# qzs634/Probabilistic-Multiplanar-Unet

Measured on AMD Instinct MI355X. Metric: 2D slices/sec fwd+bwd, 256×256×1 batch32 U-Net; Dice vs ref, higher is better.
Workload: dtype fp32; 1 GPU; c2: UNet(n_channels=1, n_classes=1, num_filters=[64, 128, 256, 512, 1024]), 256x256x1 slices, fwd+BCE+bwd+clip(0.1)+SGD(0.9) per step, fp32; global_batch=32, per_gpu_batch=32, parallelism=dp1

## Files before the change

include/pmunet_hip.h:

```cpp
#ifndef PMUNET_HIP_H
#define PMUNET_HIP_H
#include <stddef.h>
#ifdef __cplusplus
extern "C" {
#endif

#define PMU_ABI_VERSION 1

enum { PMU_OK = 0, PMU_ERR_ARG = 1001 };

enum {
  PMU_SRC_RAW = 0,
  PMU_SRC_BNRELU = 1,
  PMU_SRC_BNBWD = 2
};
enum { PMU_POOL_NONE = 0, PMU_POOL_MAX2 = 1, PMU_POOL_AVG2CEIL = 2 };
enum { PMU_DT_X_BF16 = 1, PMU_DT_Z_BF16 = 2 };

typedef struct pmu_src {
  const float* x;
  const float* z;
  const float* coef;
  int mode, pool;
  int C, H, W;
  int off_h, off_w;
  int dtype;
} pmu_src;

typedef struct pmu_frame {
  pmu_src src[2];
  int nsrc;
  int N, H, W;
} pmu_frame;

size_t pmu_conv3x3_wgrad_ws(int N, int H, int W, int Cin, int Cout);
int pmu_conv3x3_wgrad(const pmu_frame* dz, const pmu_frame* act, int Cout, float* dw,
                      float* ws, size_t ws_bytes, void* stream);

size_t pmu_conv3x3_packed_size_wino(int Cout, int Cin, int dgrad);
int pmu_conv3x3_pack_wino(const float* w, int Cout, int Cin, int dgrad, float* wp, void* stream);
int pmu_conv3x3_tiles_wino(int N, int H, int W);
int pmu_conv3x3_fwd_wino(const pmu_frame* in, const float* wp, const float* bias, int Cout, float* z,
                         float* part, float* tee, void* stream);
int pmu_conv3x3_dgrad_wino(const pmu_frame* dz, const float* wp, int Cin, int Csplit, float* dx0, float* dx1,
                           float* tee, void* stream);
size_t pmu_conv3x3_packed_size_wino2h(int Cout, int Cin, int dgrad);
int pmu_conv3x3_pack_wino2h(const float* w, int Cout, int Cin, int dgrad, float* wp, void* stream);
int pmu_conv3x3_tiles_wino2h(int N, int H, int W);
int pmu_conv3x3_fwd_wino2h(const float* xt, int Cin, int N, int H, int W, const float* wp, const float* bias,
                           int Cout, float* z, float* part, void* stream);
int pmu_conv3x3_dgrad_wino2h(const float* dzt, int Cout, int N, int H, int W, const float* wp, int Cin,
                             int Csplit, float* dx0, float* dx1, void* stream);
int pmu_conv3x3_dgrad_wino2h_bnr(const float* dzt, int Cout, int N, int H, int W, const float* wp, int Cin,
                                 float* dx, const float* z, const float* coef, const float* mean,
                                 const float* invstd, float* part, void* stream);
size_t pmu_conv3x3_packed_size_wino4(int Cout, int Cin, int dgrad);
int pmu_conv3x3_pack_wino4(const float* w, int Cout, int Cin, int dgrad, float* wp, void* stream);
int pmu_conv3x3_tiles_wino4(int N, int H, int W);
int pmu_conv3x3_dgrad_wino4(const float* dzt, int Cout, int N, int H, int W, const float* wp, int Cin,
                            int Csplit, float* dx0, float* dx1, void* stream);
int pmu_conv3x3_dgrad_wino4_bnr(const float* dzt, int Cout, int N, int H, int W, const float* wp, int Cin,
                                float* dx, const float* z, const float* coef, const float* mean,
                                const float* invstd, float* part, void* stream);
size_t pmu_conv3x3_wgrad_ws_wino(int N, int H, int W, int Cin, int Cout);
int pmu_conv3x3_wgrad_wino(const float* dzt, const float* xt, int N, int H, int W, int Cout, int Cin,
                           float* dw, float* ws, size_t ws_bytes, void* stream);

size_t pmu_conv3x3_packed_size_bf16(int Cout, int Cin, int dgrad);
int pmu_conv3x3_pack_bf16(const float* w, int Cout, int Cin, int dgrad, unsigned short* wp, void* stream);
int pmu_conv3x3_tiles(int N, int H, int W);
int pmu_conv3x3_fwd_bf16(const pmu_frame* in, const unsigned short* wp, const float* bias, int Cout,
                         float* z, float* part, unsigned short* tee, void* stream);
int pmu_conv3x3_dgrad_bf16(const pmu_frame* dz, const unsigned short* wp, int Cin, int Csplit,
                           float* dx0, float* dx1, unsigned short* tee, void* stream);

size_t pmu_conv3x3_packed_size_raw(int Cout, int Cin, int dgrad);
int pmu_conv3x3_pack_raw(const float* w, int Cout, int Cin, int dgrad, unsigned short* wp, void* stream);
int pmu_conv3x3_fwd_raw(const unsigned short* xt, int Cp, int N, int H, int W, const unsigned short* wp,
                        const float* bias, int Cout, float* z, float* part, void* stream);
int pmu_conv3x3_tiles_raw(int N, int H, int W, int Cout);
int pmu_conv3x3_dgrad_raw(const unsigned short* dzt, int Cp, int N, int H, int W, const unsigned short* wp,
                          int Cin, int Csplit, float* dx0, float* dx1, void* stream);
int pmu_conv3x3_dma_ok(int H, int W, int Cp, int NOUT, int split);
int pmu_conv3x3_tiles_dma(int N, int H, int W, int Cout, int Cp);
size_t pmu_conv3x3_packed_size_dma(int Cout, int Cin, int dgrad);
int pmu_conv3x3_pack_dma(const float* w, int Cout, int Cin, int dgrad, unsigned short* wp, void* stream);
int pmu_conv3x3_fwd_dma(const unsigned short* xt, int Cp, int N, int H, int W, const unsigned short* wp,
                        const float* bias, int Cout, float* z, float* part, void* stream);
int pmu_conv3x3_dgrad_dma(const unsigned short* dzt, int Cp, int N, int H, int W, const unsigned short* wp,
                          int Cin, int Csplit, float* dx0, float* dx1, void* stream);
int pmu_conv3x3_dgrad_dma_x1b(const unsigned short* dzt, int Cp, int N, int H, int W, const unsigned short* wp,
                              int Cin, int Csplit, float* dx0, float* dx1, unsigned short* dx1b, void* stream);
int pmu_conv3x3_dgrad_dma_x1b_sum(const unsigned short* dzt, int Cp, int N, int H, int W, const unsigned short* wp,
                                  int Cin, int Csplit, float* dx0, unsigned short* dx1b, float* part, void* stream);
size_t pmu_convT2x2_dbias_rows_ws(int Cout);
int pmu_convT2x2_dbias_rows(const float* part, int R, long long ld, int Cout, float* dbias, float* ws, void* stream);
int pmu_conv3x3_dgrad_dma_bnr(const unsigned short* dzt, int Cp, int N, int H, int W, const unsigned short* wp,
                              int Cin, float* dx, const float* z, const float* coef, const float* mean,
                              const float* invstd, float* part, void* stream);
int pmu_conv3x3_dgrad_dma_dxb(const unsigned short* dzt, int Cp, int N, int H, int W, const unsigned short* wp,
                              int Cin, int Csplit, unsigned short* dx0, float* dx1, void* stream);
// ... 230 lines not shown
```

probabilistic-multiplanar-unet_amd/csrc/conv3x3_wino2h.hip:

```cpp
#include <string.h>
#include <stdlib.h>
#include "pmu_common.h"
#include "pmu_lds.h"

namespace {

constexpr int TX = 8, TY = 8;
constexpr int OW = 2 * TX, OH = 2 * TY;
constexpr int HW = OW + 2, HH = OH + 2;
constexpr int BK = 8;
constexpr int GP = 20;
constexpr int ROWF = 208;
constexpr int ROWU = ROWF / 4;
constexpr int A_FLOATS = HH * ROWF;
[[maybe_unused]] constexpr int NC = 16;
constexpr int NCP = 16;
constexpr int A_UNITS = A_FLOATS / 4;

__host__ __device__ constexpr int u_swz(int row) { return (row >> 2) & 3; }

template <int CO_>
struct W2Cfg {
  static constexpr int CO = CO_;
  static constexpr int NT = 16 * CO_;
  static constexpr int NW = NT / 64;
  static constexpr int U_FLOATS = BK * CO_ * NCP;
  static constexpr int STAGE = A_FLOATS + U_FLOATS;
  static constexpr int NGL = (A_UNITS + NT - 1) / NT;
  static constexpr int UGL = (U_FLOATS / 4 + NT - 1) / NT;
  static constexpr int RED_FLOATS = NW * 16 * 2;
  static constexpr int XB_FLOATS = NW * 2 * 4 * 64;
  static_assert(U_FLOATS % (4 * 64) == 0, "U of whole wave DMA instructions");
  static_assert(XB_FLOATS <= STAGE, "exchange round fits a stage");
  static_assert((2 * STAGE + RED_FLOATS) * 4 <= 160 * 1024, "LDS");
};

struct W2Args {
  const float* x;
  const float* wp;
  const float* bias;
  float* out0;
  float* out1;
  float* part;
  int H, W, KC, NOUT, split, bw, bh, nco, cpb;
  int N;
  const float* bz;
  const float* bcoef;
  const float* bmean;
  const float* binv;
};

__device__ __forceinline__ void wino2_u(const float (&g)[3][3], float (&u)[16]) {
  float t[4][3];
  for (int b = 0; b < 3; ++b) {
    t[0][b] = g[0][b];
    t[1][b] = 0.5f * (g[0][b] + g[1][b] + g[2][b]);
    t[2][b] = 0.5f * (g[0][b] - g[1][b] + g[2][b]);
    t[3][b] = g[2][b];
  }
  for (int a = 0; a < 4; ++a) {
    u[4 * a + 0] = t[a][0];
    u[4 * a + 1] = 0.5f * (t[a][0] + t[a][1] + t[a][2]);
    u[4 * a + 2] = 0.5f * (t[a][0] - t[a][1] + t[a][2]);
    u[4 * a + 3] = t[a][2];
  }
}

template <int CO>
__device__ __forceinline__ void pack_wino2h_body(const float* __restrict__ w, int Cout, int Cin, int dgrad,
                                                 float* __restrict__ wp, int bid, int nblk) {
  const int NOUT = dgrad ? Cin : Cout, KC = dgrad ? Cout : Cin;
  const int nch = (KC + BK - 1) / BK, ncob = (NOUT + CO - 1) / CO;
  const long long total = (long long)ncob * nch * BK * CO;
  for (long long e = (long long)bid * blockDim.x + threadIdx.x; e < total; e += (long long)nblk * blockDim.x) {
    const int col = (int)(e % CO);
    long long r = e / CO;
    const int kl = (int)(r % BK); r /= BK;
    const int ch = (int)(r % nch);
    const int jb = (int)(r / nch);
    const int j = jb * CO + col, k = ch * BK + kl;
    float g[3][3];
    for (int a = 0; a < 3; ++a)
      for (int b = 0; b < 3; ++b) {
        float v = 0.f;
        if (j < NOUT && k < KC)
          v = dgrad ? w[((long long)k * Cin + j) * 9 + (2 - a) * 3 + (2 - b)] : w[((long long)j * Cin + k) * 9 + a * 3 + b];
        g[a][b] = v;
      }
    float u[16];
    wino2_u(g, u);
    float* dst = wp + (((long long)jb * nch + ch) * BK + kl) * (CO * NCP) + col * NCP;
    const int sw = u_swz(kl * CO + col);
    for (int q = 0; q < 4; ++q)
      *reinterpret_cast<float4*>(dst + 4 * (q ^ sw)) = make_float4(u[4 * q], u[4 * q + 1], u[4 * q + 2], u[4 * q + 3]);
  }
}
template <int CO>
// ... 259 lines not shown
        float* rowp = dst + (long long)((long long)n * a.H + min(hh, a.H - 1)) * a.W * ld;
#pragma unroll
        for (int q = 0; q < 2; ++q) {
          const int ww = ow + q;
          const float v = P[2 * p + q] + xv[2 * p + q] + bias;
          const bool ok = jok && hh < a.H && ww < a.W;
          if (!DGRAD) {
            const float m = ok ? v : 0.f;
            s1 += m;
            s2 = fmaf(m, m, s2);
          } else if (BNR) {
            const float zz = zt[2 * p + q];
            const float g = (ok && fmaf(zz, bsc, bsh) > 0.f) ? v : 0.f;
            s1 += g;
            s2 = fmaf(g, (zz - bmu) * bis, s2);
          }
          if (!ok) continue;
          PMU_DCHECK((((long long)n * a.H + hh) * a.W + ww) < (long long)a.N * a.H * a.W && j < a.NOUT, PMU_DBG_OUTPUT);
          rowp[(unsigned)(ww * ld)] = v;
        }
      }
    }
  }
  if (a.part) {
    s1 += __shfl_xor(s1, 16, 64);
    s2 += __shfl_xor(s2, 16, 64);
    s1 += __shfl_xor(s1, 32, 64);
    s2 += __shfl_xor(s2, 32, 64);
    if (lane < 16) {
      red[(wave * 16 + lane) * 2 + 0] = s1;
      red[(wave * 16 + lane) * 2 + 1] = s2;
    }
    __syncthreads();
    if (tid < CO) {
      const int jj = j0 + tid, cgg = tid >> 5, hf = (tid >> 4) & 1, l = tid & 15;
      if (jj < a.NOUT) {
        float t1 = 0.f, t2 = 0.f;
#pragma unroll
        for (int g = 0; g < 4; ++g) {
          const int wv = g + 4 * hf + 8 * cgg;
          t1 += red[(wv * 16 + l) * 2 + 0];
          t2 += red[(wv * 16 + l) * 2 + 1];
        }
        PMU_DCHECK(spatial < (long long)a.N * a.bh * a.bw, PMU_DBG_WORKSPACE);
        a.part[((long long)spatial * 2 + 0) * a.NOUT + jj] = t1;
        a.part[((long long)spatial * 2 + 1) * a.NOUT + jj] = t2;
      }
    }
  }
  __syncthreads();
}

struct W2Block {
  int n, h0, w0, cob0, spatial, nchunks, npass;
  unsigned gin, gzero;
};

template <bool DGRAD, bool BNR, int CH, int CO_, bool P64>
__device__ __forceinline__ void wino2h_main(const W2Args& a, const W2Block& B, const unsigned (&goff)[W2Cfg<CO_>::NGL],
                                            float* smem) {
  using C = W2Cfg<CO_>;
  constexpr int CO = C::CO, NT = C::NT, NGL = C::NGL, UGL = C::UGL, U_FLOATS = C::U_FLOATS, STAGE = C::STAGE;
  float* red = smem + 2 * STAGE;
  const int tid = threadIdx.x, lane = tid & 63, wave = tid >> 6;
  const int nchunks = B.nchunks, total = B.npass * nchunks;
  const float* wsrc = a.wp + (long long)B.cob0 * nchunks * U_FLOATS;
  const unsigned uoff = 16u * tid;
  const int wave_off = wave * 256;
  const unsigned gin = B.gin;
#define PMU_FETCH2(GI, BUF)                                                                                 \
  {                                                                                                        \
    const int p_ = (GI) / nchunks;                                                                         \
    const int c_ = (GI) - p_ * nchunks;                                                                    \
    const int cs_ = ((B.cob0 + p_) & 1) ? nchunks - 1 - c_ : c_;                                           \
    const int k0_ = cs_ * BK;                                                                              \
    PMU_DCHECK(k0_ + BK <= a.KC, PMU_DBG_OPERAND);                                                         \
    float* b_ = (BUF);                                                                                     \
    const char* xb_ = reinterpret_cast<const char*>(a.x + k0_);                                            \
    _Pragma("unroll") for (int r = 0; r < NGL; ++r)                                                        \
      if ((gin >> r) & 1u) PMU_GLDS(xb_ + goff[r], b_ + 4 * (r * NT) + wave_off)                           \
    const char* s_ = reinterpret_cast<const char*>(wsrc + ((long long)p_ * nchunks + cs_) * U_FLOATS) + uoff; \
    float* d_ = b_ + A_FLOATS + wave_off;                                                                  \
    _Pragma("unroll") for (int r = 0; r < UGL; ++r)                                                        \
      if (r * NT * 4 + (wave + 1) * 256 <= U_FLOATS) PMU_GLDS(s_ + 16 * NT * r, d_ + 4 * NT * r)          \
  }
  const int t = lane & 15, kk = lane >> 4, tg = wave & 3, cg = wave >> 3;
  const int pbase = 2 * (2 * tg + (t >> 3)) * ROWF + GP * (t & 7) + 2 * kk;
  const int ubase = A_FLOATS + (2 * kk * CO + 32 * cg + t) * NCP;
  static_assert(CO % 16 == 0, "u_swz of every row a lane reads is (t >> 2) & 3");
  const unsigned uoff0 = 4u * ubase + 16u * ((2 * CH) ^ ((t >> 2) & 3));
  f32x4 acc[2][8];
#pragma unroll
  for (int h = 0; h < 2; ++h)
#pragma unroll
    for (int c = 0; c < 8; ++c) acc[h][c] = f32x4{0.f, 0.f, 0.f, 0.f};

  PMU_FETCH2(0, smem)
  asm volatile("s_waitcnt vmcnt(0)" ::: "memory");
  __syncthreads();
  for (int p = 0; p < B.npass; ++p) {
    const int j0 = (B.cob0 + p) * CO;
    const int jb = j0 + 32 * cg + 16 * CH + t;
    const float bias = (!DGRAD && a.bias && jb < a.NOUT) ? a.bias[jb] : 0.f;
    int gi = p * nchunks;
    for (int ch = 0; ch < nchunks; ++ch, ++gi) {
      float* cur = smem + (gi & 1) * STAGE;
      if (gi + 1 < total) PMU_FETCH2(gi + 1, smem + ((gi + 1) & 1) * STAGE)
      const unsigned pa = lds_addr(cur + pbase), ua0 = lds_addr(cur) + uoff0, ua1 = ua0 ^ 16u;
      if constexpr (P64) {
        w2_pair<CH, CO>(pa, ua0, acc);
      } else {
        w2_step<CH>(pa, ua0, ua1, acc);
        w2_step<CH>(pa + 4, ua0 + CO * NCP * 4, ua1 + CO * NCP * 4, acc);
      }
      asm volatile("s_waitcnt vmcnt(0)" ::: "memory");
      __syncthreads();
    }
    int ne = B.n, h0e = B.h0, w0e = B.w0;
    asm volatile("" : "+s"(ne), "+s"(h0e), "+s"(w0e));
    float* xb = smem + ((gi - 1) & 1) * STAGE;
    wino2h_epilogue<DGRAD, BNR, CH, CO>(a, ne, h0e, w0e, j0, B.spatial, acc, xb, red, bias);
    if (p + 1 < B.npass) {
#pragma unroll
      for (int r = 0; r < NGL; ++r)
        if ((B.gzero >> r) & 1u) *reinterpret_cast<float4*>(xb + 4 * (r * NT + tid)) = make_float4(0.f, 0.f, 0.f, 0.f);
      __syncthreads();
    }
#pragma unroll
    for (int h = 0; h < 2; ++h)
#pragma unroll
      for (int c = 0; c < 8; ++c) acc[h][c] = f32x4{0.f, 0.f, 0.f, 0.f};
  }
#undef PMU_FETCH2
}

template <bool DGRAD, bool BNR, int CO_, bool P64 = true>
__global__ __launch_bounds__(16 * CO_, CO_ == 32 ? 4 : 1) void conv3x3_wino2h_kernel(W2Args a) {
  using C = W2Cfg<CO_>;
  constexpr int NT = C::NT, NGL = C::NGL, STAGE = C::STAGE;
  __shared__ __attribute__((aligned(64))) float smem[2 * STAGE + C::RED_FLOATS];
  static_assert(A_FLOATS % 16 == 0 && STAGE % 16 == 0, "U rows 64-B aligned (ua1 = ua0 ^ 16)");
  const int tid = threadIdx.x;
  const int lb = pmu_xcd_block(blockIdx.x, gridDim.x);
  const int ncog = (a.nco + a.cpb - 1) / a.cpb;
  W2Block B;
  B.cob0 = (lb % ncog) * a.cpb;
  int sp = lb / ncog;
  B.spatial = sp;
  const int bx = sp % a.bw; sp /= a.bw;
  const int by = sp % a.bh;
  B.n = sp / a.bh;
  B.h0 = by * OH;
  B.w0 = bx * OW;
  const int KC = a.KC;
  B.nchunks = KC / BK;
  B.npass = a.cpb < a.nco - B.cob0 ? a.cpb : a.nco - B.cob0;
  PMU_DCHECK(B.n < a.N && B.cob0 < a.nco, PMU_DBG_GRID);
  unsigned goff[NGL];
  unsigned gin = 0u, gzero = 0u;
#pragma unroll
  for (int r = 0; r < NGL; ++r) {
    const int u = r * NT + tid;
    const int hr = u / ROWU, wu = u - hr * ROWU;
    const int g = wu / 5, w5 = wu - 5 * g;
    const int px = 2 * g + (w5 >> 1);
    const bool data = u < A_UNITS && w5 < 4 && px < HW;
    const int h = B.h0 - 1 + hr, w = B.w0 - 1 + px;
    const bool in = data && h >= 0 && w >= 0 && h < a.H && w < a.W;
    goff[r] = in ? (unsigned)(((((long long)B.n * a.H + h) * a.W + w) * KC + 4 * (w5 & 1)) * 4) : 0u;
    PMU_DCHECK(!in || (((long long)B.n * a.H + h) * a.W + w) < (long long)a.N * a.H * a.W, PMU_DBG_OPERAND);
    gin |= in ? (1u << r) : 0u;
    gzero |= (data && !in) ? (1u << r) : 0u;
    if (data && !in) {
      *reinterpret_cast<float4*>(smem + 4 * u) = make_float4(0.f, 0.f, 0.f, 0.f);
      *reinterpret_cast<float4*>(smem + STAGE + 4 * u) = make_float4(0.f, 0.f, 0.f, 0.f);
    }
  }
  B.gin = gin;
  B.gzero = gzero;
  if ((tid >> 8) & 1) wino2h_main<DGRAD, BNR, 1, CO_, P64>(a, B, goff, smem);
  else wino2h_main<DGRAD, BNR, 0, CO_, P64>(a, B, goff, smem);
}

static int w2h_co() {
  static const int v = pmu_variant_int("PMU_WINO2H_CO", 64) == 32 ? 32 : 64;
  return v;
}

int launch_wino2h(const float* x, int KC, int N, int H, int W, const float* wp, const float* bias, int NOUT,
                  float* out0, float* out1, int split, float* part, bool dgrad, void* stream,
                 const float* bz = nullptr, const float* bcoef = nullptr, const float* bmean = nullptr,
                 const float* binv = nullptr) {
  const pmu_wino_call c{x, KC, N, H, W, wp, bias, NOUT, out0, out1, split, part, bz, bcoef, bmean, binv};
  const int CO = w2h_co();
  return pmu_wino_launch<W2Args>(c, OW, OH, BK, CO, "PMU_WINO2H_CPB", "PMU_WINO2H_MINWG",
                                 [&](const W2Args& a, long long, dim3 grid) {
    hipStream_t st = (hipStream_t)stream;
    const bool bnr = dgrad && bz;
#ifdef PMU_EXPERIMENTS
    static const int b32 = pmu_variant_int("PMU_WINO2H_B32", 0);
    if (CO == 32 && bnr) hipLaunchKernelGGL((conv3x3_wino2h_kernel<true, true, 32, false>), grid, dim3(512), 0, st, a);
    else if (CO == 32 && dgrad) hipLaunchKernelGGL((conv3x3_wino2h_kernel<true, false, 32, false>), grid, dim3(512), 0, st, a);
    else if (CO == 32) hipLaunchKernelGGL((conv3x3_wino2h_kernel<false, false, 32, false>), grid, dim3(512), 0, st, a);
    else if (b32 && bnr) hipLaunchKernelGGL((conv3x3_wino2h_kernel<true, true, 64, false>), grid, dim3(1024), 0, st, a);
    else if (b32 && dgrad) hipLaunchKernelGGL((conv3x3_wino2h_kernel<true, false, 64, false>), grid, dim3(1024), 0, st, a);
    else if (b32) hipLaunchKernelGGL((conv3x3_wino2h_kernel<false, false, 64, false>), grid, dim3(1024), 0, st, a);
    else
#endif
    if (bnr) hipLaunchKernelGGL((conv3x3_wino2h_kernel<true, true, 64>), grid, dim3(1024), 0, st, a);
    else if (dgrad) hipLaunchKernelGGL((conv3x3_wino2h_kernel<true, false, 64>), grid, dim3(1024), 0, st, a);
    else hipLaunchKernelGGL((conv3x3_wino2h_kernel<false, false, 64>), grid, dim3(1024), 0, st, a);
    PMU_CHECK_LAUNCH();
    return (int)PMU_OK;
  });
}

}

extern "C" int pmu_conv3x3_tiles_wino2h(int N, int H, int W) { return N * pmu_cdiv(H, OH) * pmu_cdiv(W, OW); }

extern "C" size_t pmu_conv3x3_packed_size_wino2h(int Cout, int Cin, int dgrad) {
  const int NOUT = dgrad ? Cin : Cout, KC = dgrad ? Cout : Cin;
  const int CO = w2h_co();
  return (size_t)pmu_cdiv(NOUT, CO) * pmu_cdiv(KC, BK) * (BK * CO * NCP) * sizeof(float);
}

extern "C" int pmu_conv3x3_pack_wino2h(const float* w, int Cout, int Cin, int dgrad, float* wp, void* stream) {
  PMU_REQUIRE(w && wp && Cout > 0 && Cin > 0);
  const long long total = (long long)pmu_conv3x3_packed_size_wino2h(Cout, Cin, dgrad) / sizeof(float) / NCP;
  const int blocks = (int)((total + 255) / 256 < 4096 ? (total + 255) / 256 : 4096);
  hipStream_t st = (hipStream_t)stream;
  const unsigned segs = (unsigned)(pmu_cdiv(Cout, w2h_co()) * pmu_cdiv(Cin, BK));
#ifdef PMU_EXPERIMENTS
  if (w2h_co() == 32 && !dgrad)
    hipLaunchKernelGGL(pack_wino2h_fwd_kernel<32>, dim3(segs), dim3(256), 0, st, w, Cout, Cin, wp);
  else if (w2h_co() == 32)
    hipLaunchKernelGGL(pack_wino2h_kernel<32>, dim3(blocks), dim3(256), 0, st, w, Cout, Cin, dgrad, wp);
  else
#endif
  if (!dgrad) hipLaunchKernelGGL(pack_wino2h_fwd_kernel<64>, dim3(segs), dim3(256), 0, st, w, Cout, Cin, wp);
  else hipLaunchKernelGGL(pack_wino2h_kernel<64>, dim3(blocks), dim3(256), 0, st, w, Cout, Cin, dgrad, wp);
  PMU_CHECK_LAUNCH();
  return PMU_OK;
}

extern "C" int pmu_conv3x3_fwd_wino2h(const float* xt, int Cin, int N, int H, int W, const float* wp, const float* bias,
                                      int Cout, float* z, float* part, void* stream) {
  return launch_wino2h(xt, Cin, N, H, W, wp, bias, Cout, z, nullptr, Cout, part, false, stream);
}

extern "C" int pmu_conv3x3_dgrad_wino2h(const float* dzt, int Cout, int N, int H, int W, const float* wp, int Cin,
                                        int Csplit, float* dx0, float* dx1, void* stream) {
  PMU_REQUIRE(Csplit > 0 && Csplit <= Cin && (Csplit == Cin || dx1));
  return launch_wino2h(dzt, Cout, N, H, W, wp, nullptr, Cin, dx0, dx1, Csplit, nullptr, true, stream);
}

extern "C" int pmu_conv3x3_dgrad_wino2h_bnr(const float* dzt, int Cout, int N, int H, int W, const float* wp, int Cin,
                                            float* dx, const float* z, const float* coef, const float* mean,
                                            const float* invstd, float* part, void* stream) {
  PMU_REQUIRE(z && coef && mean && invstd && part);
  return launch_wino2h(dzt, Cout, N, H, W, wp, nullptr, Cin, dx, nullptr, Cin, part, true, stream, z, coef, mean,
                       invstd);
}

static int pack_wino2h_grid(int Cout, int Cin, int dgrad) {
  if (!dgrad) return pmu_cdiv(Cout, w2h_co()) * pmu_cdiv(Cin, BK);
  const long long total = (long long)pmu_conv3x3_packed_size_wino2h(Cout, Cin, dgrad) / sizeof(float) / NCP;
  return (int)((total + 255) / 256 < 4096 ? (total + 255) / 256 : 4096);
}

extern "C" int pmu_conv3x3_pack_wino2h_blocks(int Cout, int Cin, int dgrad) { return pack_wino2h_grid(Cout, Cin, dgrad); }

extern "C" int pmu_conv3x3_pack_wino2h_multi(const pmu_pack_job* jobs, int njobs, int blocks, int dgrad, void* stream) {
// ... 7 lines not shown
```

probabilistic-multiplanar-unet_amd/csrc/conv3x3_wino4.hip:

```cpp
#include <string.h>
#include <stdlib.h>
#include <utility>
#include "pmu_common.h"
#include "pmu_lds.h"

namespace {

constexpr int TX = 8, TY = 8;
constexpr int OW = 4 * TX, OH = 4 * TY;
constexpr int HW = OW + 2, HH = OH + 2;
constexpr int BK = 8;
constexpr int GP = 36;
constexpr int ROWF = 312;
constexpr int ROWU = ROWF / 4;
constexpr int A_FLOATS = HH * ROWF;
constexpr int CO = 32;
constexpr int NC = 36;
constexpr int U_FLOATS = BK * CO * NC;
constexpr int STAGE = A_FLOATS + U_FLOATS;
constexpr int NT = 512;
constexpr int A_UNITS = A_FLOATS / 4;
constexpr int NGL = (A_UNITS + NT - 1) / NT;
constexpr int UGL = (U_FLOATS / 4 + NT - 1) / NT;
constexpr int RED_FLOATS = 8 * 16 * 2;
// ... 543 lines not shown
  if (a.tc > 0) {
    const int gsz = a.ts * a.tc, g = lb / gsz, i = lb - g * gsz;
    const int gpr = ncog / a.tc;
    cg = (g % gpr) * a.tc + i % a.tc;
    sp = (g / gpr) * a.ts + i / a.tc;
  } else {
    cg = lb % ncog;
    sp = lb / ncog;
  }
  B.cob0 = cg * a.cpb;
  B.spatial = sp;
  const int bx = sp % a.bw; sp /= a.bw;
  const int by = sp % a.bh;
  B.n = sp / a.bh;
  B.h0 = by * OH;
  B.w0 = bx * OW;
  const int KC = a.KC;
  B.nchunks = KC / BK;
  B.npass = a.cpb < a.nco - B.cob0 ? a.cpb : a.nco - B.cob0;
  PMU_DCHECK(B.n < a.N && B.cob0 < a.nco, PMU_DBG_GRID);

  unsigned goff[NGL];
  unsigned gin = 0u, gzero = 0u;
#pragma unroll
  for (int r = 0; r < NGL; ++r) {
    const int u = r * NT + tid;
    const int hr = u / ROWU, wu = u - hr * ROWU;
    const int g = wu / 9, w9 = wu - 9 * g;
    const int px = 4 * g + (w9 >> 1);
    const bool data = u < A_UNITS && w9 < 8 && px < HW;
    const int h = B.h0 - 1 + hr, w = B.w0 - 1 + px;
    const bool in = data && h >= 0 && w >= 0 && h < a.H && w < a.W;
    goff[r] = in ? (unsigned)(((((long long)B.n * a.H + h) * a.W + w) * KC + 4 * (w9 & 1)) * 4) : 0u;
    PMU_DCHECK(!in || (((long long)B.n * a.H + h) * a.W + w) < (long long)a.N * a.H * a.W, PMU_DBG_OPERAND);
    gin |= in ? (1u << r) : 0u;
    gzero |= (data && !in) ? (1u << r) : 0u;
    if (data && !in) {
      *reinterpret_cast<float4*>(smem + 4 * u) = make_float4(0.f, 0.f, 0.f, 0.f);
      *reinterpret_cast<float4*>(smem + STAGE + 4 * u) = make_float4(0.f, 0.f, 0.f, 0.f);
    }
  }
  B.gin = gin;
  B.gzero = gzero;
  if (a.prio && (tid >> 8)) __builtin_amdgcn_s_setprio(1);
  if (tid >> 8) wino4_main<DGRAD, BNR, 1, PM>(a, B, goff, smem);
  else wino4_main<DGRAD, BNR, 0, PM>(a, B, goff, smem);
}

int launch_wino4(const float* x, int KC, int N, int H, int W, const float* wp, const float* bias, int NOUT,
                 float* out0, float* out1, int split, float* part, bool dgrad, void* stream,
                 const float* bz = nullptr, const float* bcoef = nullptr, const float* bmean = nullptr,
                 const float* binv = nullptr) {
  const pmu_wino_call c{x, KC, N, H, W, wp, bias, NOUT, out0, out1, split, part, bz, bcoef, bmean, binv};
  return pmu_wino_launch<W4Args>(c, OW, OH, BK, CO, "PMU_WINO4_CPB", "PMU_WINO4_MINWG",
                                 [&](W4Args& a, long long spatial, dim3 grid) {
    static const int pf = pmu_variant_int("PMU_WINO4_PF", 0);
    static const int b32 = pmu_variant_int("PMU_WINO4_B32", 0);
    const int pm = pf ? 1 : b32 ? 0 : 2;
    static const int prio = pmu_variant_int("PMU_WINO4_PRIO", 0);
    a.prio = prio;
    static const int grp = pmu_variant_int("PMU_WINO4_GROUP", 1);
    if (grp) {
      const int ncog = pmu_cdiv(a.nco, a.cpb);
      const int tc = ncog < 8 ? ncog : 8, ts = 32 / tc;
      if (ncog % tc == 0 && spatial % ts == 0 && tc > 1 && ts > 1) { a.tc = tc; a.ts = ts; }
    }
    hipStream_t st = (hipStream_t)stream;
#ifdef PMU_EXPERIMENTS
    if (dgrad && bz && pm == 0) hipLaunchKernelGGL((conv3x3_wino4_kernel<true, true, 0>), grid, dim3(NT), 0, st, a);
    else if (dgrad && bz) hipLaunchKernelGGL((conv3x3_wino4_kernel<true, true, 2>), grid, dim3(NT), 0, st, a);
    else if (dgrad && pm == 1) hipLaunchKernelGGL((conv3x3_wino4_kernel<true, false, 1>), grid, dim3(NT), 0, st, a);
    else if (dgrad && pm == 0) hipLaunchKernelGGL((conv3x3_wino4_kernel<true, false, 0>), grid, dim3(NT), 0, st, a);
    else if (dgrad) hipLaunchKernelGGL((conv3x3_wino4_kernel<true, false, 2>), grid, dim3(NT), 0, st, a);
    else if (pm == 1) hipLaunchKernelGGL((conv3x3_wino4_kernel<false, false, 1>), grid, dim3(NT), 0, st, a);
    else if (pm == 0) hipLaunchKernelGGL((conv3x3_wino4_kernel<false, false, 0>), grid, dim3(NT), 0, st, a);
    else hipLaunchKernelGGL((conv3x3_wino4_kernel<false, false, 2>), grid, dim3(NT), 0, st, a);
#else
    (void)pm;
    if (dgrad && bz) hipLaunchKernelGGL((conv3x3_wino4_kernel<true, true, 2>), grid, dim3(NT), 0, st, a);
    else if (dgrad) hipLaunchKernelGGL((conv3x3_wino4_kernel<true, false, 2>), grid, dim3(NT), 0, st, a);
    else return (int)PMU_ERR_ARG;
#endif
    PMU_CHECK_LAUNCH();
    return (int)PMU_OK;
  });
}

}

extern "C" int pmu_conv3x3_tiles_wino4(int N, int H, int W) { return N * pmu_cdiv(H, OH) * pmu_cdiv(W, OW); }

extern "C" size_t pmu_conv3x3_packed_size_wino4(int Cout, int Cin, int dgrad) {
  const int NOUT = dgrad ? Cin : Cout, KC = dgrad ? Cout : Cin;
  return (size_t)pmu_cdiv(NOUT, CO) * pmu_cdiv(KC, BK) * U_FLOATS * sizeof(float);
}

extern "C" int pmu_conv3x3_pack_wino4(const float* w, int Cout, int Cin, int dgrad, float* wp, void* stream) {
  PMU_REQUIRE(w && wp && Cout > 0 && Cin > 0);
  const int NOUT = dgrad ? Cin : Cout, KC = dgrad ? Cout : Cin;
  const unsigned segs = (unsigned)(pmu_cdiv(NOUT, CO) * pmu_cdiv(KC, BK));
  hipLaunchKernelGGL(pack_wino4_kernel, dim3(segs), dim3(256), 0, (hipStream_t)stream, w, Cout, Cin, dgrad, wp);
  PMU_CHECK_LAUNCH();
  return PMU_OK;
}

#ifdef PMU_EXPERIMENTS
extern "C" int pmu_conv3x3_fwd_wino4(const float* xt, int Cin, int N, int H, int W, const float* wp, const float* bias,
                                     int Cout, float* z, float* part, void* stream) {
// ... 31 lines not shown
```

probabilistic-multiplanar-unet_amd/csrc/pmu_common.h:

```cpp
#pragma once
#include <hip/hip_runtime.h>
#include <stdint.h>
#include <stdlib.h>
#include <string.h>
#include "../../include/pmunet_hip.h"

typedef float f32x16 __attribute__((ext_vector_type(16)));

#define PMU_CHECK_LAUNCH()                          \
  do {                                              \
    hipError_t e__ = hipGetLastError();             \
    if (e__ != hipSuccess) return (int)e__;         \
  } while (0)
#define PMU_REQUIRE(cond) \
  do {                    \
    if (!(cond)) return PMU_ERR_ARG; \
  } while (0)

static inline int pmu_cdiv(long long a, long long b) { return (int)((a + b - 1) / b); }
static inline unsigned grid_for(long long n) {
  const long long g = (n + 255) / 256;
  return (unsigned)(g > 8192 ? 8192 : g < 1 ? 1 : g);
}
constexpr int HEAD_KMAX = 8;
// ... 12 lines not shown
  }
  red[tid] = ((a0 + a1) + a2) + a3;
  __syncthreads();
  double t = 0.0;
  if (tid < 64)
    for (int p = 0; p < 16; ++p) t += red[p * 64 + tid];
  return t;
}

static inline int pmu_num_cus() {
  static const int cus = [] {
    int dev = 0, n = 256;
    if (hipGetDevice(&dev) != hipSuccess || hipDeviceGetAttribute(&n, hipDeviceAttributeMultiprocessorCount, dev) != hipSuccess)
      n = 256;
    return n;
  }();
  return cus;
}

static inline const char* pmu_variant_env(const char* name) {
#ifdef PMU_EXPERIMENTS
  return getenv(name);
#else
  (void)name;
  return nullptr;
#endif
}
static inline int pmu_env_int(const char* name, int dflt) {
  const char* e = getenv(name);
  return e ? atoi(e) : dflt;
}
static inline int pmu_variant_int(const char* name, int dflt) {
  const char* e = pmu_variant_env(name);
  return e ? atoi(e) : dflt;
}

template <class F>
static inline int pmu_image_chunks(int N, long long bytes_per_image, F&& f) {
  PMU_REQUIRE(bytes_per_image > 0 && bytes_per_image < (1LL << 32));
  const long long per = ((1LL << 32) - 1) / bytes_per_image;
  for (long long n0 = 0; n0 < N; n0 += per) {
    const int nn = (int)(N - n0 < per ? N - n0 : per);
    const int rc = f((int)n0, nn);
    if (rc) return rc;
  }
  return 0;
}

static inline int pmu_wino_cpb(int nco, long long spatial, int cpb_env, int min_wg) {
  if (cpb_env > 0) return cpb_env < nco ? cpb_env : nco;
  int cpb = 1;
  while (cpb * 2 <= nco && spatial * pmu_cdiv(nco, cpb * 2) >= min_wg) cpb *= 2;
  return cpb;
}

struct pmu_wino_call {
  const float* x;
  int KC, N, H, W;
  const float* wp;
  const float* bias;
  int NOUT;
  float* out0;
  float* out1;
  int split;
  float* part;
  const float* bz;
  const float* bcoef;
  const float* bmean;
  const float* binv;
};
template <class Args, class F>
static inline int pmu_wino_launch(const pmu_wino_call& c, int OW, int OH, int BK, int CO, const char* cpb_name,
                                  const char* minwg_name, F&& launch) {
  PMU_REQUIRE(c.x && c.wp && c.out0 && c.KC > 0 && c.KC % BK == 0 && c.NOUT > 0 && c.N > 0 && c.H > 0 && c.W > 0);
  const long long img_bytes = (long long)c.H * c.W * (c.KC > c.NOUT ? c.KC : c.NOUT) * 4;
  if ((long long)c.N * img_bytes >= (1LL << 32)) {
    const long long tiles = (long long)pmu_cdiv(c.W, OW) * pmu_cdiv(c.H, OH);
    return pmu_image_chunks(c.N, img_bytes, [&](int n0, int nn) {
      const long long px = (long long)n0 * c.H * c.W;
      pmu_wino_call s = c;
      s.N = nn;
      s.x = c.x + px * c.KC;
      s.out0 = c.out0 + px * c.split;
      s.out1 = c.out1 ? c.out1 + px * (c.NOUT - c.split) : nullptr;
      s.part = c.part ? c.part + (long long)n0 * tiles * 2 * c.NOUT : nullptr;
      s.bz = c.bz ? c.bz + px * c.NOUT : nullptr;
      return pmu_wino_launch<Args>(s, OW, OH, BK, CO, cpb_name, minwg_name, launch);
    });
  }
  Args a;
  memset(&a, 0, sizeof(a));
  a.x = c.x; a.wp = c.wp; a.bias = c.bias; a.out0 = c.out0; a.out1 = c.out1; a.part = c.part;
  a.H = c.H; a.W = c.W; a.KC = c.KC; a.NOUT = c.NOUT; a.split = c.split;
  a.N = c.N;
  a.bz = c.bz; a.bcoef = c.bcoef; a.bmean = c.bmean; a.binv = c.binv;
  a.bw = pmu_cdiv(c.W, OW);
  a.bh = pmu_cdiv(c.H, OH);
  a.nco = pmu_cdiv(c.NOUT, CO);
  const long long spatial = (long long)a.bw * a.bh * c.N;
  static const int cpb_env = pmu_env_int(cpb_name, 0);
  static const int min_wg = pmu_env_int(minwg_name, 1024);
  a.cpb = pmu_wino_cpb(a.nco, spatial, cpb_env, min_wg);
  const long long blocks = (long long)pmu_cdiv(a.nco, a.cpb) * spatial;
  PMU_REQUIRE(blocks < (1LL << 31));
  return launch(a, spatial, dim3((unsigned)blocks));
}

__device__ __forceinline__ int pmu_job_of(const pmu_pack_job* jobs, int njobs, int bid) {
  int j = 0;
  while (j + 1 < njobs && jobs[j + 1].block0 <= bid) ++j;
  return j;
}

__device__ __forceinline__ int pmu_xcd_block(int bid, int nb) {
  const int x = bid & 7, q = nb >> 3, r = nb & 7;
  return x * q + (x < r ? x : r) + (bid >> 3);
}
__device__ __forceinline__ int pmu_cdiv_dev(int a, int b) { return (a + b - 1) / b; }

__device__ __forceinline__ f32x16 mfma_f32_32x32x2(float a, float b, f32x16 c) {
  return __builtin_amdgcn_mfma_f32_32x32x2f32(a, b, c, 0, 0, 0);
}
__device__ __forceinline__ int acc_row(int r, int lane) { return (r & 3) + 8 * (r >> 2) + 4 * (lane >> 5); }

__device__ __forceinline__ float pmu_bf16_f32(unsigned short u) { return __uint_as_float((unsigned)u << 16); }
__device__ __forceinline__ unsigned short pmu_f32_bf16(float v) { return __builtin_bit_cast(unsigned short, (__bf16)v); }
__device__ __forceinline__ float pmu_round_bf16(float v) { return pmu_bf16_f32(pmu_f32_bf16(v)); }
typedef __bf16 bf16x8 __attribute__((ext_vector_type(8)));
typedef short s16x4 __attribute__((ext_vector_type(4)));
typedef __attribute__((address_space(3))) s16x4 lds_s16x4;

__device__ __forceinline__ int pmu_swap1(int v) { return __builtin_amdgcn_update_dpp(0, v, 0xB1, 0xF, 0xF, true); }
__device__ __forceinline__ unsigned pmu_swap1(unsigned v) { return (unsigned)pmu_swap1((int)v); }
__device__ __forceinline__ float pmu_swap1(float v) {
  return __builtin_bit_cast(float, pmu_swap1(__builtin_bit_cast(int, v)));
}

template <int CTRL>
__device__ __forceinline__ float pmu_dpp(float v) {
  return __builtin_bit_cast(float, __builtin_amdgcn_update_dpp(0, __builtin_bit_cast(int, v), CTRL, 0xF, 0xF, true));
}
__device__ __forceinline__ float pmu_group_sum(float v, int CQ) {
  if (CQ >= 2) v += pmu_dpp<0xB1>(v);
  if (CQ >= 4) v += pmu_dpp<0x4E>(v);
  if (CQ >= 8) v += pmu_dpp<0x141>(v);
  if (CQ >= 16) v += pmu_dpp<0x140>(v);
  for (int o = 16; o < CQ; o <<= 1) v += __shfl_xor(v, o, 64);
  return v;
}
__device__ __forceinline__ float4 pmu_ld4(const float* p) { return *reinterpret_cast<const float4*>(p); }
__device__ __forceinline__ float4 pmu_ld4(const unsigned short* p) {
  const uint2 u = *reinterpret_cast<const uint2*>(p);
  return make_float4(__uint_as_float(u.x << 16), __uint_as_float(u.x & 0xffff0000u), __uint_as_float(u.y << 16),
                     __uint_as_float(u.y & 0xffff0000u));
}
__device__ __forceinline__ float pmu_ld1(const float* p) { return *p; }
__device__ __forceinline__ float pmu_ld1(const unsigned short* p) { return pmu_bf16_f32(*p); }

// ... 225 lines not shown
```

probabilistic-multiplanar-unet_amd/pmu_hip/_lib.py:

```python
from __future__ import annotations

import ctypes
import os
from ctypes import POINTER, c_double, c_float, c_int, c_longlong, c_size_t, c_void_p

import torch

LIB_NAME = {"debug": "libpmunet_hip_debug.so", "exp": "libpmunet_hip_exp.so",
            "prev": "libpmunet_hip_prev.so"}.get(os.environ.get("PMU_LIB", ""), "libpmunet_hip.so")
LIB_PATH = os.path.join(os.path.dirname(os.path.abspath(__file__)), LIB_NAME)
HEADER_PATH = os.path.normpath(
    os.path.join(os.path.dirname(os.path.abspath(__file__)), "..", "..", "include", "pmunet_hip.h"))
EXP_HEADER_PATH = os.path.join(os.path.dirname(HEADER_PATH), "pmunet_hip_experiments.h")
EXP_LIB_PATH = os.path.join(os.path.dirname(os.path.abspath(__file__)), "libpmunet_hip_exp.so")

PMU_OK = 0
PMU_ERR_ARG = 1001
SRC_RAW, SRC_BNRELU, SRC_BNBWD = 0, 1, 2
POOL_NONE, POOL_MAX2, POOL_AVG2CEIL = 0, 1, 2
DT_X_BF16, DT_Z_BF16 = 1, 2


class PmuSrc(ctypes.Structure):
    _fields_ = [("x", c_void_p), ("z", c_void_p), ("coef", c_void_p), ("mode", c_int), ("pool", c_int),
                ("C", c_int), ("H", c_int), ("W", c_int), ("off_h", c_int), ("off_w", c_int), ("dtype", c_int)]


class PmuFrame(ctypes.Structure):
    _fields_ = [("src", PmuSrc * 2), ("nsrc", c_int), ("N", c_int), ("H", c_int), ("W", c_int)]


class PmuPackJob(ctypes.Structure):
    _fields_ = [("w", c_void_p), ("dst", c_void_p), ("Cout", c_int), ("Cin", c_int), ("block0", c_int),
                ("nblocks", c_int)]


class PmuSgdChunk(ctypes.Structure):
    _fields_ = [("tensor", c_int), ("len", c_int), ("start", c_longlong)]


_FP = POINTER(PmuFrame)
SIGNATURES = {
    "pmu_conv3x3_tiles": (c_int, [c_int, c_int, c_int]),
    "pmu_conv3x3_wgrad_ws": (c_size_t, [c_int, c_int, c_int, c_int, c_int]),
    "pmu_conv3x3_wgrad": (c_int, [_FP, _FP, c_int, c_void_p, c_void_p, c_size_t, c_void_p]),
    "pmu_conv3x3_packed_size_wino": (c_size_t, [c_int, c_int, c_int]),
    "pmu_conv3x3_pack_wino": (c_int, [c_void_p, c_int, c_int, c_int, c_void_p, c_void_p]),
    "pmu_conv3x3_tiles_wino": (c_int, [c_int, c_int, c_int]),
    "pmu_conv3x3_fwd_wino": (c_int, [_FP, c_void_p, c_void_p, c_int, c_void_p, c_void_p, c_void_p, c_void_p]),
    "pmu_conv3x3_dgrad_wino": (c_int, [_FP, c_void_p, c_int, c_int, c_void_p, c_void_p, c_void_p, c_void_p]),
    "pmu_conv3x3_packed_size_wino2h": (c_size_t, [c_int, c_int, c_int]),
    "pmu_conv3x3_pack_wino2h": (c_int, [c_void_p, c_int, c_int, c_int, c_void_p, c_void_p]),
    "pmu_conv3x3_tiles_wino2h": (c_int, [c_int, c_int, c_int]),
    "pmu_conv3x3_fwd_wino2h": (c_int, [c_void_p, c_int, c_int, c_int, c_int, c_void_p, c_void_p, c_int, c_void_p,
                                       c_void_p, c_void_p]),
    "pmu_conv3x3_dgrad_wino2h": (c_int, [c_void_p, c_int, c_int, c_int, c_int, c_void_p, c_int, c_int, c_void_p,
                                         c_void_p, c_void_p]),
    "pmu_conv3x3_packed_size_wino4": (c_size_t, [c_int, c_int, c_int]),
    "pmu_conv3x3_pack_wino4": (c_int, [c_void_p, c_int, c_int, c_int, c_void_p, c_void_p]),
    "pmu_conv3x3_tiles_wino4": (c_int, [c_int, c_int, c_int]),
    "pmu_conv3x3_dgrad_wino4": (c_int, [c_void_p, c_int, c_int, c_int, c_int, c_void_p, c_int, c_int, c_void_p,
                                        c_void_p, c_void_p]),
    "pmu_conv3x3_wgrad_ws_wino": (c_size_t, [c_int, c_int, c_int, c_int, c_int]),
    "pmu_conv3x3_wgrad_wino": (c_int, [c_void_p, c_void_p, c_int, c_int, c_int, c_int, c_int, c_void_p, c_void_p,
                                       c_size_t, c_void_p]),
    "pmu_conv3x3_packed_size_bf16": (c_size_t, [c_int, c_int, c_int]),
    "pmu_conv3x3_pack_bf16": (c_int, [c_void_p, c_int, c_int, c_int, c_void_p, c_void_p]),
    "pmu_conv3x3_fwd_bf16": (c_int, [_FP, c_void_p, c_void_p, c_int, c_void_p, c_void_p, c_void_p, c_void_p]),
    "pmu_conv3x3_dgrad_bf16": (c_int, [_FP, c_void_p, c_int, c_int, c_void_p, c_void_p, c_void_p, c_void_p]),
    "pmu_conv3x3_packed_size_raw": (c_size_t, [c_int, c_int, c_int]),
    "pmu_conv3x3_tiles_raw": (c_int, [c_int, c_int, c_int, c_int]),
    "pmu_conv3x3_pack_raw": (c_int, [c_void_p, c_int, c_int, c_int, c_void_p, c_void_p]),
    "pmu_conv3x3_fwd_raw": (c_int, [c_void_p, c_int, c_int, c_int, c_int, c_void_p, c_void_p, c_int, c_void_p,
                                    c_void_p, c_void_p]),
    "pmu_conv3x3_dgrad_raw": (c_int, [c_void_p, c_int, c_int, c_int, c_int, c_void_p, c_int, c_int, c_void_p,
                                      c_void_p, c_void_p]),
    "pmu_frame_to_bf16": (c_int, [_FP, c_int, c_void_p, c_void_p]),
    "pmu_frame_to_f32": (c_int, [_FP, c_void_p, c_void_p]),
    "pmu_frame_to_f32_ld": (c_int, [_FP, c_void_p, c_int, c_void_p]),
    "pmu_frame_to_bf16_ld": (c_int, [_FP, c_int, c_void_p, c_int, c_void_p]),
    "pmu_frame_pool_skip_ok": (c_int, [_FP]),
    "pmu_frame_to_bf16_pool_skip": (c_int, [_FP, c_void_p, c_void_p, c_int, c_void_p]),
    "pmu_frame_to_f32_pool_skip": (c_int, [_FP, c_void_p, c_void_p, c_int, c_void_p]),
    "pmu_conv3x3_wgrad_ws_bf16": (c_size_t, [c_int, c_int, c_int, c_int, c_int]),
    "pmu_conv3x3_wgrad_bf16": (c_int, [c_void_p, c_void_p, c_int, c_int, c_int, c_int, c_int, c_void_p, c_void_p,
                                       c_size_t, c_void_p]),
    "pmu_convT2x2_wgrad_ws_bf16": (c_size_t, [c_int, c_int, c_int, c_int, c_int]),
    "pmu_convT2x2_wgrad_bf16": (c_int, [c_void_p, c_void_p, c_void_p, c_int, c_int, c_int, c_int, c_int, c_int,
                                        c_int, c_int, c_int, c_void_p, c_void_p, c_void_p, c_size_t, c_void_p]),
    "pmu_occupancy_conv3x3_raw": (c_int, [POINTER(c_int)]),
    "pmu_occupancy_wgrad3x3_bf16": (c_int, [POINTER(c_int)]),
    "pmu_conv_first_fwd": (c_int, [POINTER(c_void_p), c_int, c_int, c_int, c_int, c_void_p, c_void_p, c_int,
                                   c_void_p, c_void_p, c_void_p]),
    "pmu_conv_first_tiles": (c_int, [c_int, c_int, c_int]),
    "pmu_conv_first_wgrad_ws": (c_size_t, [c_int, c_int, c_int, c_int, c_int]),
    "pmu_conv_first_wgrad": (c_int, [_FP, POINTER(c_void_p), c_int, c_int, c_void_p, c_void_p, c_size_t,
                                     c_void_p]),
    "pmu_colsum_f64": (c_int, [c_void_p, c_int, c_int, c_void_p, c_int, c_void_p]),
    "pmu_colsum_groups": (c_int, [c_int]),
    "pmu_bn_fwd_finalize": (c_int, [c_void_p, c_int, c_int, c_double, c_void_p, c_void_p, c_float, c_float,
                                    c_void_p, c_void_p, c_void_p, c_void_p, c_void_p, c_void_p, c_void_p]),
    "pmu_bn_eval_coef": (c_int, [c_void_p, c_void_p, c_void_p, c_void_p, c_float, c_int, c_void_p, c_void_p]),
    "pmu_bn_bwd_reduce": (c_int, [c_void_p, c_void_p, c_void_p, c_void_p, c_void_p, c_int, c_int, c_void_p,
                                  c_void_p]),
    "pmu_bn_bwd_tiles": (c_int, [c_int, c_int]),
    "pmu_bn_bwd_finalize": (c_int, [c_void_p, c_int, c_int, c_double, c_void_p, c_void_p, c_void_p, c_void_p,
# ... 307 lines not shown
```

Measured before the change: 716.5 slices/s.

## Let wino2h workgroups process multiple images per block to cut launch oversubscription

Adds an images-per-block (ipb) dimension to the Winograd F(2x2) kernel. Each workgroup now loops over several batch images as well as output-channel passes, and prefetches the next image's input tile across the image boundary. The goal is to shrink the grid when there are far more workgroups than needed for occupancy, for example on the small deep layers with batch 32, and so amortize per-block setup and weight reuse. In exchange it reduces parallelism and may lengthen the tail. The ipb value is chosen automatically against the min-workgroup threshold and can be overridden through an environment variable.

```diff
diff --git a/include/pmunet_hip.h b/include/pmunet_hip.h
--- a/include/pmunet_hip.h
+++ b/include/pmunet_hip.h
@@ -47,6 +47,7 @@
 size_t pmu_conv3x3_packed_size_wino2h(int Cout, int Cin, int dgrad);
 int pmu_conv3x3_pack_wino2h(const float* w, int Cout, int Cin, int dgrad, float* wp, void* stream);
 int pmu_conv3x3_tiles_wino2h(int N, int H, int W);
+int pmu_conv3x3_wino2h_launch_blocks(int N, int H, int W, int Nout, int* cpb, int* ipb);
 int pmu_conv3x3_fwd_wino2h(const float* xt, int Cin, int N, int H, int W, const float* wp, const float* bias,
                            int Cout, float* z, float* part, void* stream);
 int pmu_conv3x3_dgrad_wino2h(const float* dzt, int Cout, int N, int H, int W, const float* wp, int Cin,
diff --git a/probabilistic-multiplanar-unet_amd/csrc/conv3x3_wino2h.hip b/probabilistic-multiplanar-unet_amd/csrc/conv3x3_wino2h.hip
--- a/probabilistic-multiplanar-unet_amd/csrc/conv3x3_wino2h.hip
+++ b/probabilistic-multiplanar-unet_amd/csrc/conv3x3_wino2h.hip
@@ -43,6 +43,7 @@
   float* out1;
   float* part;
   int H, W, KC, NOUT, split, bw, bh, nco, cpb;
+  int ipb;
   int N;
   const float* bz;
   const float* bcoef;
@@ -408,7 +409,7 @@
 }
 
 struct W2Block {
-  int n, h0, w0, cob0, spatial, nchunks, npass;
+  int n, h0, w0, cob0, spatial, nchunks, npass, nimg;
   unsigned gin, gzero;
 };
 
@@ -419,23 +420,21 @@
   constexpr int CO = C::CO, NT = C::NT, NGL = C::NGL, UGL = C::UGL, U_FLOATS = C::U_FLOATS, STAGE = C::STAGE;
   float* red = smem + 2 * STAGE;
   const int tid = threadIdx.x, lane = tid & 63, wave = tid >> 6;
-  const int nchunks = B.nchunks, total = B.npass * nchunks;
+  const int nchunks = B.nchunks, nq = B.nimg * B.npass;
   const float* wsrc = a.wp + (long long)B.cob0 * nchunks * U_FLOATS;
   const unsigned uoff = 16u * tid;
   const int wave_off = wave * 256;
   const unsigned gin = B.gin;
-#define PMU_FETCH2(GI, BUF)                                                                                 \
+#define PMU_FETCH2(IM, P, C, BUF)                                                                           \
   {                                                                                                        \
-    const int p_ = (GI) / nchunks;                                                                         \
-    const int c_ = (GI) - p_ * nchunks;                                                                    \
-    const int cs_ = ((B.cob0 + p_) & 1) ? nchunks - 1 - c_ : c_;                                           \
+    const int cs_ = ((B.cob0 + (P)) & 1) ? nchunks - 1 - (C) : (C);                                        \
     const int k0_ = cs_ * BK;                                                                              \
-    PMU_DCHECK(k0_ + BK <= a.KC, PMU_DBG_OPERAND);                                                         \
+    PMU_DCHECK(k0_ + BK <= a.KC && B.n + (IM) < a.N, PMU_DBG_OPERAND);                                     \
     float* b_ = (BUF);                                                                                     \
-    const char* xb_ = reinterpret_cast<const char*>(a.x + k0_);                                            \
+    const char* xb_ = reinterpret_cast<const char*>(a.x + (long long)(IM) * a.H * a.W * a.KC + k0_);       \
     _Pragma("unroll") for (int r = 0; r < NGL; ++r)                                                        \
       if ((gin >> r) & 1u) PMU_GLDS(xb_ + goff[r], b_ + 4 * (r * NT) + wave_off)                           \
-    const char* s_ = reinterpret_cast<const char*>(wsrc + ((long long)p_ * nchunks + cs_) * U_FLOATS) + uoff; \
+    const char* s_ = reinterpret_cast<const char*>(wsrc + ((long long)(P) * nchunks + cs_) * U_FLOATS) + uoff; \
     float* d_ = b_ + A_FLOATS + wave_off;                                                                  \
     _Pragma("unroll") for (int r = 0; r < UGL; ++r)                                                        \
       if (r * NT * 4 + (wave + 1) * 256 <= U_FLOATS) PMU_GLDS(s_ + 16 * NT * r, d_ + 4 * NT * r)          \
@@ -451,17 +450,21 @@
 #pragma unroll
     for (int c = 0; c < 8; ++c) acc[h][c] = f32x4{0.f, 0.f, 0.f, 0.f};
 
-  PMU_FETCH2(0, smem)
+  PMU_FETCH2(0, 0, 0, smem)
   asm volatile("s_waitcnt vmcnt(0)" ::: "memory");
   __syncthreads();
-  for (int p = 0; p < B.npass; ++p) {
+  for (int q = 0; q < nq; ++q) {
+    const int im = q / B.npass, p = q - im * B.npass;
+    const int pn = p + 1 < B.npass ? p + 1 : 0, imn = pn ? im : im + 1;
     const int j0 = (B.cob0 + p) * CO;
     const int jb = j0 + 32 * cg + 16 * CH + t;
     const float bias = (!DGRAD && a.bias && jb < a.NOUT) ? a.bias[jb] : 0.f;
-    int gi = p * nchunks;
+    int gi = q * nchunks;
     for (int ch = 0; ch < nchunks; ++ch, ++gi) {
       float* cur = smem + (gi & 1) * STAGE;
-      if (gi + 1 < total) PMU_FETCH2(gi + 1, smem + ((gi + 1) & 1) * STAGE)
+      float* nxt = smem + ((gi + 1) & 1) * STAGE;
+      const bool same = ch + 1 < nchunks;
+      if (same || q + 1 < nq) PMU_FETCH2(same ? im : imn, same ? p : pn, same ? ch + 1 : 0, nxt)
       const unsigned pa = lds_addr(cur + pbase), ua0 = lds_addr(cur) + uoff0, ua1 = ua0 ^ 16u;
       if constexpr (P64) {
         w2_pair<CH, CO>(pa, ua0, acc);
@@ -472,11 +475,11 @@
       asm volatile("s_waitcnt vmcnt(0)" ::: "memory");
       __syncthreads();
     }
-    int ne = B.n, h0e = B.h0, w0e = B.w0;
-    asm volatile("" : "+s"(ne), "+s"(h0e), "+s"(w0e));
+    int ne = B.n + im, h0e = B.h0, w0e = B.w0, spe = B.spatial + im * a.bh * a.bw;
+    asm volatile("" : "+s"(ne), "+s"(h0e), "+s"(w0e), "+s"(spe));
     float* xb = smem + ((gi - 1) & 1) * STAGE;
-    wino2h_epilogue<DGRAD, BNR, CH, CO>(a, ne, h0e, w0e, j0, B.spatial, acc, xb, red, bias);
-    if (p + 1 < B.npass) {
+    wino2h_epilogue<DGRAD, BNR, CH, CO>(a, ne, h0e, w0e, j0, spe, acc, xb, red, bias);
+    if (q + 1 < nq) {
 #pragma unroll
       for (int r = 0; r < NGL; ++r)
         if ((B.gzero >> r) & 1u) *reinterpret_cast<float4*>(xb + 4 * (r * NT + tid)) = make_float4(0.f, 0.f, 0.f, 0.f);
@@ -502,16 +505,17 @@
   W2Block B;
   B.cob0 = (lb % ncog) * a.cpb;
   int sp = lb / ncog;
-  B.spatial = sp;
   const int bx = sp % a.bw; sp /= a.bw;
   const int by = sp % a.bh;
-  B.n = sp / a.bh;
+  B.n = (sp / a.bh) * a.ipb;
+  B.nimg = a.ipb < a.N - B.n ? a.ipb : a.N - B.n;
+  B.spatial = (B.n * a.bh + by) * a.bw + bx;
   B.h0 = by * OH;
   B.w0 = bx * OW;
   const int KC = a.KC;
   B.nchunks = KC / BK;
   B.npass = a.cpb < a.nco - B.cob0 ? a.cpb : a.nco - B.cob0;
-  PMU_DCHECK(B.n < a.N && B.cob0 < a.nco, PMU_DBG_GRID);
+  PMU_DCHECK(B.n < a.N && B.nimg >= 1 && B.cob0 < a.nco, PMU_DBG_GRID);
   unsigned goff[NGL];
   unsigned gin = 0u, gzero = 0u;
 #pragma unroll
@@ -549,8 +553,9 @@
                  const float* binv = nullptr) {
   const pmu_wino_call c{x, KC, N, H, W, wp, bias, NOUT, out0, out1, split, part, bz, bcoef, bmean, binv};
   const int CO = w2h_co();
-  return pmu_wino_launch<W2Args>(c, OW, OH, BK, CO, "PMU_WINO2H_CPB", "PMU_WINO2H_MINWG",
-                                 [&](const W2Args& a, long long, dim3 grid) {
+  return pmu_wino_launch<W2Args>(c, OW, OH, BK, CO, "PMU_WINO2H_CPB", "PMU_WINO2H_IPB", "PMU_WINO2H_MINWG",
+                                 [&](W2Args& a, const pmu_wino_shape& sh, dim3 grid) {
+    a.ipb = sh.ipb;
     hipStream_t st = (hipStream_t)stream;
     const bool bnr = dgrad && bz;
 #ifdef PMU_EXPERIMENTS
@@ -575,6 +580,14 @@
 
 extern "C" int pmu_conv3x3_tiles_wino2h(int N, int H, int W) { return N * pmu_cdiv(H, OH) * pmu_cdiv(W, OW); }
 
+extern "C" int pmu_conv3x3_wino2h_launch_blocks(int N, int H, int W, int Nout, int* cpb, int* ipb) {
+  if (N <= 0 || H <= 0 || W <= 0 || Nout <= 0) return 0;
+  const pmu_wino_shape s = pmu_wino_shape_of(N, H, W, Nout, OW, OH, w2h_co(), 0, 0, 1024);
+  if (cpb) *cpb = s.cpb;
+  if (ipb) *ipb = s.ipb;
+  return s.blocks < (1LL << 31) ? (int)s.blocks : 0;
+}
+
 extern "C" size_t pmu_conv3x3_packed_size_wino2h(int Cout, int Cin, int dgrad) {
   const int NOUT = dgrad ? Cin : Cout, KC = dgrad ? Cout : Cin;
   const int CO = w2h_co();
diff --git a/probabilistic-multiplanar-unet_amd/csrc/conv3x3_wino4.hip b/probabilistic-multiplanar-unet_amd/csrc/conv3x3_wino4.hip
--- a/probabilistic-multiplanar-unet_amd/csrc/conv3x3_wino4.hip
+++ b/probabilistic-multiplanar-unet_amd/csrc/conv3x3_wino4.hip
@@ -619,8 +619,9 @@
                  const float* bz = nullptr, const float* bcoef = nullptr, const float* bmean = nullptr,
                  const float* binv = nullptr) {
   const pmu_wino_call c{x, KC, N, H, W, wp, bias, NOUT, out0, out1, split, part, bz, bcoef, bmean, binv};
-  return pmu_wino_launch<W4Args>(c, OW, OH, BK, CO, "PMU_WINO4_CPB", "PMU_WINO4_MINWG",
-                                 [&](W4Args& a, long long spatial, dim3 grid) {
+  return pmu_wino_launch<W4Args>(c, OW, OH, BK, CO, "PMU_WINO4_CPB", nullptr, "PMU_WINO4_MINWG",
+                                 [&](W4Args& a, const pmu_wino_shape& sh, dim3 grid) {
+    const long long spatial = sh.spatial;
     static const int pf = pmu_variant_int("PMU_WINO4_PF", 0);
     static const int b32 = pmu_variant_int("PMU_WINO4_B32", 0);
     const int pm = pf ? 1 : b32 ? 0 : 2;
diff --git a/probabilistic-multiplanar-unet_amd/csrc/pmu_common.h b/probabilistic-multiplanar-unet_amd/csrc/pmu_common.h
--- a/probabilistic-multiplanar-unet_amd/csrc/pmu_common.h
+++ b/probabilistic-multiplanar-unet_amd/csrc/pmu_common.h
@@ -88,6 +88,32 @@
   int cpb = 1;
   while (cpb * 2 <= nco && spatial * pmu_cdiv(nco, cpb * 2) >= min_wg) cpb *= 2;
   return cpb;
+}
+
+static inline int pmu_wino_ipb(int N, long long wg_per_image, int ipb_env, int min_wg) {
+  if (ipb_env > 0) return ipb_env < N ? ipb_env : N;
+  int ipb = 1;
+  while (ipb * 2 <= N && wg_per_image * pmu_cdiv(N, ipb * 2) >= min_wg) ipb *= 2;
+  return ipb;
+}
+
+struct pmu_wino_shape {
+  int bw, bh, nco, cpb, ipb;
+  long long spatial;
+  long long blocks;
+};
+static inline pmu_wino_shape pmu_wino_shape_of(int N, int H, int W, int NOUT, int OW, int OH, int CO, int cpb_env,
+                                               int ipb_env, int min_wg) {
+  pmu_wino_shape s;
+  s.bw = pmu_cdiv(W, OW);
+  s.bh = pmu_cdiv(H, OH);
+  s.nco = pmu_cdiv(NOUT, CO);
+  s.cpb = pmu_wino_cpb(s.nco, (long long)s.bw * s.bh * N, cpb_env, min_wg);
+  const int ncog = pmu_cdiv(s.nco, s.cpb);
+  s.ipb = pmu_wino_ipb(N, (long long)s.bw * s.bh * ncog, ipb_env, min_wg);
+  s.spatial = (long long)s.bw * s.bh * pmu_cdiv(N, s.ipb);
+  s.blocks = ncog * s.spatial;
+  return s;
 }
 
 struct pmu_wino_call {
@@ -107,7 +133,7 @@
 };
 template <class Args, class F>
 static inline int pmu_wino_launch(const pmu_wino_call& c, int OW, int OH, int BK, int CO, const char* cpb_name,
-                                  const char* minwg_name, F&& launch) {
+                                  const char* ipb_name, const char* minwg_name, F&& launch) {
   PMU_REQUIRE(c.x && c.wp && c.out0 && c.KC > 0 && c.KC % BK == 0 && c.NOUT > 0 && c.N > 0 && c.H > 0 && c.W > 0);
   const long long img_bytes = (long long)c.H * c.W * (c.KC > c.NOUT ? c.KC : c.NOUT) * 4;
   if ((long long)c.N * img_bytes >= (1LL << 32)) {
@@ -121,7 +147,7 @@
       s.out1 = c.out1 ? c.out1 + px * (c.NOUT - c.split) : nullptr;
       s.part = c.part ? c.part + (long long)n0 * tiles * 2 * c.NOUT : nullptr;
       s.bz = c.bz ? c.bz + px * c.NOUT : nullptr;
-      return pmu_wino_launch<Args>(s, OW, OH, BK, CO, cpb_name, minwg_name, launch);
+      return pmu_wino_launch<Args>(s, OW, OH, BK, CO, cpb_name, ipb_name, minwg_name, launch);
     });
   }
   Args a;
@@ -130,16 +156,13 @@
   a.H = c.H; a.W = c.W; a.KC = c.KC; a.NOUT = c.NOUT; a.split = c.split;
   a.N = c.N;
   a.bz = c.bz; a.bcoef = c.bcoef; a.bmean = c.bmean; a.binv = c.binv;
-  a.bw = pmu_cdiv(c.W, OW);
-  a.bh = pmu_cdiv(c.H, OH);
-  a.nco = pmu_cdiv(c.NOUT, CO);
-  const long long spatial = (long long)a.bw * a.bh * c.N;
   static const int cpb_env = pmu_env_int(cpb_name, 0);
+  static const int ipb_env = ipb_name ? pmu_env_int(ipb_name, 0) : 1;
   static const int min_wg = pmu_env_int(minwg_name, 1024);
-  a.cpb = pmu_wino_cpb(a.nco, spatial, cpb_env, min_wg);
-  const long long blocks = (long long)pmu_cdiv(a.nco, a.cpb) * spatial;
-  PMU_REQUIRE(blocks < (1LL << 31));
-  return launch(a, spatial, dim3((unsigned)blocks));
+  const pmu_wino_shape sh = pmu_wino_shape_of(c.N, c.H, c.W, c.NOUT, OW, OH, CO, cpb_env, ipb_env, min_wg);
+  a.bw = sh.bw; a.bh = sh.bh; a.nco = sh.nco; a.cpb = sh.cpb;
+  PMU_REQUIRE(sh.blocks < (1LL << 31));
+  return launch(a, sh, dim3((unsigned)sh.blocks));
 }
 
 __device__ __forceinline__ int pmu_job_of(const pmu_pack_job* jobs, int njobs, int bid) {
diff --git a/probabilistic-multiplanar-unet_amd/pmu_hip/_lib.py b/probabilistic-multiplanar-unet_amd/pmu_hip/_lib.py
--- a/probabilistic-multiplanar-unet_amd/pmu_hip/_lib.py
+++ b/probabilistic-multiplanar-unet_amd/pmu_hip/_lib.py
@@ -52,6 +52,7 @@
     "pmu_conv3x3_packed_size_wino2h": (c_size_t, [c_int, c_int, c_int]),
     "pmu_conv3x3_pack_wino2h": (c_int, [c_void_p, c_int, c_int, c_int, c_void_p, c_void_p]),
     "pmu_conv3x3_tiles_wino2h": (c_int, [c_int, c_int, c_int]),
+    "pmu_conv3x3_wino2h_launch_blocks": (c_int, [c_int, c_int, c_int, c_int, POINTER(c_int), POINTER(c_int)]),
     "pmu_conv3x3_fwd_wino2h": (c_int, [c_void_p, c_int, c_int, c_int, c_int, c_void_p, c_void_p, c_int, c_void_p,
                                        c_void_p, c_void_p]),
     "pmu_conv3x3_dgrad_wino2h": (c_int, [c_void_p, c_int, c_int, c_int, c_int, c_void_p, c_int, c_int, c_void_p,
```

New measurement: 722.0 slices/s (median of 6 runs). No clear change (+0.8%).
